# GiboDidact/Computational_ray_tracer

Hardware: AMD Instinct MI355X
Metric: Msamples/s (whole node) at 1920x1080; achieved HBM GB/s vs roofline (higher is better)
Workload: dtype f32; 1 GPU; BASELINE configs[1]: Cornell box 1920x1080 @ 256 spp (16x16 stratified jittered), diffuse + NEE, max depth 5, 1 quad light, 36 triangles; spp_total=256, max_depth=5, parallelism=pixel-tile shards x1 (32x32 tiles) + RCCL film reduce

## Files before the change

### computational_ray_tracer_amd/csrc/rt_device.h

```cpp
#pragma once
#include <hip/hip_runtime.h>
#include <stdint.h>

#include "rt_internal.h"
#include "rt_mathf.h"

namespace rtmi {

#define RT_DEV __device__ __forceinline__

RT_DEV void sincos_det(float x, float& s, float& c) {
    float k = __builtin_rintf(x * 0.636619772367581343f);
    float r = __builtin_fmaf(-k, 1.57079637050628662109375f, x);
    r = __builtin_fmaf(-k, -4.37113900018624283e-8f, r);
    float r2 = r * r;
    float sp = __builtin_fmaf(__builtin_fmaf(-1.9515295891e-4f, r2, 8.3321608736e-3f), r2, -1.6666654611e-1f);
    float sr = __builtin_fmaf(sp * r2, r, r);
    float cp = __builtin_fmaf(__builtin_fmaf(2.443315711809948e-5f, r2, -1.388731625493765e-3f), r2, 4.166664568298827e-2f);
    float cr = __builtin_fmaf(cp * r2, r2, __builtin_fmaf(-0.5f, r2, 1.0f));
    int q = (int)k & 3;
    s = q == 0 ? sr : (q == 1 ? cr : (q == 2 ? -sr : -cr));
    c = q == 0 ? cr : (q == 1 ? -sr : (q == 2 ? -cr : sr));
}
template <class T = rtm::TabConst>
// ... 146 lines not shown
    const uint32_t lo = (uint32_t)delta, hi = (uint32_t)(delta >> 32);
    const uint32_t lo0 = __builtin_amdgcn_readfirstlane(lo), hi0 = __builtin_amdgcn_readfirstlane(hi);
    if (__ballot(lo != lo0 || hi != hi0) == 0) {
        uint64_t d = (uint64_t)lo0 | ((uint64_t)hi0 << 32), M = 1u, P = 0u;
        for (int i = 0; d > 0; ++i, d >>= 1) {
            if (d & 1) {
                const uint64_t cm = kPcgJump.mult[i];
                M *= cm;
                P = P * cm + kPcgJump.plus[i];
            }
        }
        state = M * state + inc * P;
        return;
    }
    uint64_t accMult = 1u, accPlus = 0u;
    for (int i = 0; delta > 0; ++i, delta >>= 1) {
        if (delta & 1) {
            const uint64_t cm = kPcgJump.mult[i];
            accMult *= cm;
            accPlus = accPlus * cm + inc * kPcgJump.plus[i];
        }
    }
    state = accMult * state + accPlus;
}

RT_DEV uint64_t hash_int2(int a, int b) {
    const uint64_t m = 0xc6a4a7935bd1e995ull;
    uint64_t h = 0ull ^ (8ull * m);
    h = murmur_mix_block(h, (uint64_t)(uint32_t)a | ((uint64_t)(uint32_t)b << 32));
    return murmur_final(h);
}
RT_DEV float sobol_sample(const DevSampler& S, uint64_t a, int dimension, int randomize, uint32_t seed) {
    uint32_t v = 0;
    const uint32_t* C = S.sobol_mats + dimension * kSobolMatrixSize;
    for (int i = 0; a != 0; a >>= 1, i++)
        if (a & 1) v ^= C[i];
    if (randomize == 1) {
        v ^= seed;
    } else if (randomize == 2) {
        v = __builtin_bitreverse32(v);
        v ^= v * 0x3d20adeau;
        v += seed;
        v *= (seed >> 16) | 1u;
        v ^= v * 0x05526c56u;
        v ^= v * 0x53a22864u;
        v = __builtin_bitreverse32(v);
// ... 457 lines not shown
```

### computational_ray_tracer_amd/csrc/rt_host.cpp

```cpp
#include <algorithm>
#include <cstddef>
#include <cstdlib>
#include <cmath>
#include <cstdio>
#include <cstring>
#include <limits>
#include <queue>
#include <string>
#include <thread>
#include <utility>
#include <vector>

#include "../../include/rtmi355x.h"
#include "../data/spectra_data.h"
#include "../data/sensor_data.h"
#include "rt_devbuf.h"
#include "rt_guard.h"
#include "rt_internal.h"

using namespace rtmi;

namespace {

constexpr int kRingMax = 1 << 16;
// ... 428 lines not shown
    hipStream_t stream = nullptr;
    hipEvent_t film_done = nullptr;
};

struct Knobs {
    bool stage_events = true;
    int lanes = kDefaultLanes;
    int shadow_queue = 0;
    int shadow_dfs = 1;
    int sort_rays = 1;
    float bvh_node_cost = 2.5f;
    int bvh_max_leaf = kBvhMaxLeaf;
    float bvh_any_cost = 2.f;
    int bvh_any_leaf = 4;
    int force_amb = -1;
    int coop = 1;
    int mat_bins = 1;
    int emit_filter = 1;
    int debug_path = 0;
    int sort_dir_bits = 3, sort_org_bits = 3;
    int sort_org_major = -1;
    int sort_nee = 1, sort_nee_bits = 8;
    int hit_compact = 1;
    size_t batch_samples = 0;
    int denoise_lds = 1;
};

static Knobs read_knobs() {
    Knobs k;
    if (std::getenv("RTMI_NO_STAGE_EVENTS")) k.stage_events = false;
    if (const char* e = std::getenv("RTMI_LANES")) k.lanes = std::max(1, std::min(kLanes, std::atoi(e)));
    if (const char* e = std::getenv("RTMI_SHADOW_QUEUE")) k.shadow_queue = std::atoi(e);
    if (const char* e = std::getenv("RTMI_SHADOW_DFS")) k.shadow_dfs = std::atoi(e);
    if (const char* e = std::getenv("RTMI_SORT")) k.sort_rays = std::atoi(e);
    if (const char* e = std::getenv("RTMI_BVH_CI")) k.bvh_node_cost = (float)std::atof(e);
    if (const char* e = std::getenv("RTMI_BVH_LEAF")) k.bvh_max_leaf = std::max(1, std::min(15, std::atoi(e)));
    if (const char* e = std::getenv("RTMI_BVH_ANY")) {
        float ac;
        int al;
        if (std::sscanf(e, "%f/%d", &ac, &al) == 2) {
            k.bvh_any_cost = ac;
            k.bvh_any_leaf = std::max(1, std::min(15, al));
        }
    }
    if (const char* e = std::getenv("RTMI_FORCE_AMB")) k.force_amb = std::max(-1, std::min(30, std::atoi(e)));
    if (const char* e = std::getenv("RTMI_COOP")) k.coop = std::atoi(e) != 0;
    if (const char* e = std::getenv("RTMI_MAT_BINS")) k.mat_bins = std::atoi(e);
    if (const char* e = std::getenv("RTMI_EMIT_FILTER")) k.emit_filter = std::atoi(e);
    if (const char* e = std::getenv("RTMI_DEBUG_PATH_KERNELS")) k.debug_path = std::atoi(e) != 0;
    if (const char* e = std::getenv("RTMI_SORT_BITS")) {
        int db = 3, ob = 4, om = -1;
        const int got = std::sscanf(e, "%d/%d/%d", &db, &ob, &om);
        if (got >= 2 && db >= 0 && db <= 9 && ob >= 0 && ob <= 9 && 3 + 2 * db + 3 * ob <= 32) {
            k.sort_dir_bits = db;
            k.sort_org_bits = ob;
            if (got == 3) k.sort_org_major = om < 0 ? -1 : (om ? 1 : 0);
        }
    }
    if (const char* e = std::getenv("RTMI_SORT_NEE")) std::sscanf(e, "%d/%d", &k.sort_nee, &k.sort_nee_bits);
    k.sort_nee_bits = std::max(1, std::min(9, k.sort_nee_bits));
    if (const char* e = std::getenv("RTMI_HIT_COMPACT")) k.hit_compact = std::atoi(e) != 0;
    if (const char* e = std::getenv("RTMI_BATCH_SAMPLES")) k.batch_samples = (size_t)std::max(0L, std::atol(e));
    if (const char* e = std::getenv("RTMI_DENOISE_LDS")) k.denoise_lds = std::atoi(e) != 0;
    return k;
}

struct rt_ctx {
    float4 sort_lo{}, sort_scale{};
    int device = 0;
    int octree_build = RT_OCTREE_BUILD_DEVICE;
    hipStream_t stream = nullptr;
    std::string err;
    bool have_scene = false, have_cam = false, have_smp = false, have_film = false, have_integ = false;
    rt_camera_desc cam{};
    rt_sampler_desc smp{};
    rt_film_desc film{};
    rt_integrator_desc integ{};
    int n_tris = 0;
    std::vector<float> h_bounds;
    std::vector<int32_t> h_child, h_leaf_first, h_leaf_count, h_refs;
    rt_octree_info info{};
    bool cull = false;
    bool scene_full = false;
    DevScene dsc{};
// ... 151 lines not shown
    if (path) {
        HIPCHK(c, b.rec.reserve((size_t)kRecF4 * n));
        if (hit_d) HIPCHK(c, b.hitD.reserve(n));
    } else {
        HIPCHK(c, b.lamA.reserve(n)); HIPCHK(c, b.lamB.reserve(n));
    }
    return RT_OK;
}

static int dim_get2d(const DevSampler& S, int dim) {
    if (S.kind == 1) return dim + 2;
    if (S.kind == 2) return (dim + 1 >= kSobolDims ? 2 : dim) + 2;
    return dim;
}
static int dim_after_camera(const DevSampler& S, const DevCamera& cam) {
    int dim = S.kind == 2 ? 2 : 0;
    if (S.kind == 1) dim += 1;
    else if (S.kind == 2) dim = (dim >= kSobolDims ? 2 : dim) + 1;
    if (S.kind == 1) dim += 2;
    if ((cam.type == RT_CAMERA_PERSPECTIVE && cam.lens_radius > 0) || cam.type > RT_CAMERA_PINHOLE)
        dim = dim_get2d(S, dim);
    return dim;
}

hipEvent_t ev_get(rt_ctx* c) {
    if (!c->pool.empty()) {
        hipEvent_t e = c->pool.back();
        c->pool.pop_back();
        return e;
    }
    hipEvent_t e;
    hipEventCreate(&e);
    return e;
}
void ev_mark(rt_ctx* c, hipStream_t st, int stage, hipEvent_t a) {
    if (!a) return;
    hipEvent_t b = ev_get(c);
    hipEventRecord(b, st);
    c->pending.push_back({a, b, stage});
}
hipEvent_t ev_start(rt_ctx* c, hipStream_t st) {
    if (!c->knobs.stage_events) return nullptr;
    hipEvent_t a = ev_get(c);
    hipEventRecord(a, st);
    return a;
}
// ... 330 lines not shown
    }
    const bool dyn = c->dsc.qcap != 1;
    const int lean = c->dsc.full ? 2 : 1;
    const bool shq = c->dsc.qcap != 1 && !c->dsc.full;
    if (shq)
        for (int l = 0; l < lanes; ++l)
            if ((rc = ensure_shadow_workspace(c, c->ws[l].b, ncap))) return rc;
    const bool nee = c->dsc.full && c->dsc.n_lights > 0;
    if (nee)
        for (int l = 0; l < lanes; ++l)
            if ((rc = ensure_nee_workspace(c, c->ws[l].b, nmax * (size_t)nee_stride(c->dsc.n_lights), ncap))) return rc;
    const bool bins = nee && c->dsc.qcap != 1 && kn.mat_bins;
    const int grid = c->grid;
    auto lstream = [&](int l) { return l == 0 ? st : c->ws[l].stream; };
    if (lanes > 1) {
        HIPCHK(c, hipEventRecord(c->ws[0].film_done, st));
        for (int l = 1; l < lanes; ++l) HIPCHK(c, hipStreamWaitEvent(c->ws[l].stream, c->ws[0].film_done, 0));
    }
    const size_t qs = ncap;
    const bool records = c->dsc.qcap != 1;
    const size_t rec_fs = records ? 1 : nmax;
    const unsigned rec_ss = records ? (unsigned)kRecF4 : 1u;
    const int rec_rng8 = !records && lean == 1 ? 1 : 0;
    int last_film = -1;
    for (int g0 = ib; g0 < ie; g0 += B * lanes) {
        int nIdx[kLanes] = {0}, cur[kLanes] = {0}, nSq[kLanes] = {0}, Sq[kLanes] = {0};
        for (int l = 0; l < lanes; ++l) {
            int b0 = g0 + l * B;
            if (b0 >= ie) break;
            Work& w = c->ws[l];
            const Batch& b = w.b;
            hipStream_t s = lstream(l);
            const RecView rv{b.rec.get(), rec_fs, rec_ss, rec_rng8};
            nIdx[l] = std::min(B, ie - b0);
            int nS = nIdx[l] * n_work;
            nSq[l] = nS;
            Sq[l] = shard_stride(nS, nsh);
            SampleIds ids = sample_ids(work, n_work, b0);
            GenOut go{b.rayO(), b.rayD(), nullptr, nullptr, b.pdfA.get(), b.pdfB.get(), rv, lean, 1};
            go.zero = w.qcount.get();
            hipEvent_t e0 = ev_start(c, s);
            HIPCHK(c, launch_generate(s, grid, nS, ids, cam, smp, fd, go));
            ev_mark(c, s, ST_GEN, e0);
        }
        for (int depth = 0; depth <= c->integ.max_depth; ++depth) {
            if (depth == c->integ.max_depth && depth > 0 && !c->dsc.full) break;
            for (int l = 0; l < lanes && nIdx[l] > 0; ++l) {
                Work& w = c->ws[l];
                const Batch& b = w.b;
                hipStream_t s = lstream(l);
                const RecView rv{b.rec.get(), rec_fs, rec_ss, rec_rng8};
                SampleIds ids = sample_ids(work, n_work, g0 + l * B);
                int nxt = cur[l] ^ 1;
                const float4* cO = b.rayO() + 2 * (size_t)cur[l] * qs;
                const float4* cD = cO + 1;
                int* qc_cur = w.qcount.get() + kQRegion * cur[l];
                int* qc_nxt = w.qcount.get() + kQRegion * nxt;
                const bool efilter = kn.emit_filter && c->dsc.full && depth == c->integ.max_depth && depth > 0 &&
                                     c->dsc.n_emit_tris >= 0;
                if (efilter) HIPCHK(c, hipMemsetAsync(qc_nxt, 0, kQRegion * sizeof(int), s));
                hipEvent_t e0;
                QueueView qv = depth == 0 ? QueueView{nullptr, Sq[l], nSq[l], nsh}
                                          : QueueView{qc_cur + kQLen, Sq[l], 0, nsh};
                const DevScene dsl = lane_scene(c, w);
                if (efilter) {
                    const EmitIO eio{qv, cO, b.rayO() + 2 * (size_t)nxt * qs, qc_nxt + kQLen};
                    e0 = ev_start(c, s);
                    HIPCHK(c, launch_emitter_filter(s, grid, dsl, eio));
                    ev_mark(c, s, ST_FILTER, e0);
                    cO = eio.nO;
                    cD = cO + 1;
                    qv = QueueView{qc_nxt + kQLen, Sq[l], 0, nsh};
                }
                TraceIO tio{cO, cD, qv, 0, b.hitB.get(), b.hitPrim.get(), dyn ? qc_cur + kQTraceTicket : nullptr, 1};
                if (depth > 0 && !efilter) tio.zero = qc_nxt;
                const bool hitc = kn.hit_compact && c->dsc.qcap == 1 && !c->dsc.full && depth > 0;
                if (hitc) {
                    tio.hq_d = b.hitD.get();
                    tio.hq_len = qc_cur + kQShadowLen;
                }
                if (c->dsc.qcap != 1) {
                    tio.fb_pos = w.tfb.get();
                    tio.fb_len = qc_cur + kQTraceFallback;
                }
                const NeeSlots ns = nee ? b.nee : NeeSlots{};
                BinIO bio{qv, b.hitPrim.get(), {}, qc_cur + kQBinLen};
                for (int cl = 0; cl < kMatClasses; ++cl) bio.idx[cl] = ns.bin[cl];
                if (depth == 0) { bio.rayO = cO; bio.rec = rv; }
                if (sort_rays && depth > 0 && !efilter) {
                    SortRaysIO so{b.sQKey.get(), b.sS.get(), b.sKeys.get(), b.sKeysAlt.get(), b.sVals.get(),
                                  b.sValsAlt.get(), b.sTemp.get(), kn.sort_dir_bits, kn.sort_org_bits, qc_cur + kQLen,
                                  Sq[l]};
                    e0 = ev_start(c, s);
                    HIPCHK(c, launch_sort_rays(s, so));
                    ev_mark(c, s, ST_SORT, e0);
                    tio.perm = b.sS.get();
                    tio.so = b.sRay.get();
                    cO = tio.so; cD = cO + 1;
                }
                e0 = ev_start(c, s);
                HIPCHK(c, launch_trace_closest(s, grid, c->dsc.qcap, dsl, tio, d_ctr));
                if (tio.fb_pos && !c->dsc.coop_ok)
                    HIPCHK(c, launch_trace_fallback(s, grid, c->dsc.qcap, dsl, tio, d_ctr));
                ev_mark(c, s, ST_TRACE, e0);
                PathIO pio{};
                pio.lean = lean;
                pio.rayO = cO; pio.rayD = cD; pio.q = qv;
                pio.hitB = b.hitB.get(); pio.hitPrim = b.hitPrim.get();
                if (hitc) {
                    pio.q = QueueView{tio.hq_len, Sq[l], 0, nsh};
                    pio.hq_d = tio.hq_d;
                }
                pio.nO =b.rayO() + 2 * (size_t)nxt * qs; pio.nD = pio.nO + 1;
                pio.nCount = qc_nxt + kQLen;
                pio.rec = rv; pio.pdfA = b.pdfA.get(); pio.pdfB = b.pdfB.get();
                pio.depth = depth; pio.max_depth = c->integ.max_depth;
                pio.dim = -1;
                if (lean == 1) {
                    pio.dim = dim_after_camera(smp, cam);
                    for (int d = 0; d < depth; ++d) pio.dim = dim_get2d(smp, dim_get2d(smp, pio.dim));
                }
                pio.ticket = dyn ? qc_cur + kQShadeTicket : nullptr;
                if (sort_rays && depth < c->integ.max_depth) {
                    pio.nkey.key = b.sQKey.get();
                    pio.nkey.lo = c->sort_lo;
                    pio.nkey.scale = c->sort_scale;
                    pio.nkey.dir_bits = kn.sort_dir_bits;
                    pio.nkey.org_bits = kn.sort_org_bits;
                    pio.nkey.org_major = kn.sort_org_major >= 0 ? kn.sort_org_major : (c->dsc.full ? 0 : 1);
                }
                ShadowQueueIO sqio{};
                if (shq) {
                    sqio.shO = b.shO.get(); sqio.shD = b.shD.get(); sqio.shLA = b.shLA.get(); sqio.shLB = b.shLB.get();
                    sqio.shCount = qc_cur + kQShadowLen;
                    sqio.shTicket = qc_cur + kQShadowTicket;
                    sqio.defer = kn.shadow_queue ? 0 : 1;
                }
                NeeIO nio{};
                const bool sort_nee = nee && sort_rays && kn.sort_nee;
                if (nee)
                    nio = NeeIO{b.neeRec.get(), ns.queue, qc_cur + kQShadowLen, qc_cur + kQShadowTicket, ns.fallback,
                                qc_cur + kQNeeFallback, sort_nee ? ns.key : nullptr, c->sort_lo, c->sort_scale,
                                kn.sort_nee_bits};
// ... 2140 lines not shown
```

### computational_ray_tracer_amd/csrc/rt_internal.h

```cpp
#pragma once
#include <hip/hip_runtime.h>
#include <stdint.h>

#include <vector>

namespace rtmi {

static const int kSpecN = 471;
static const int kF1Max = 128;

struct DevSpectra {
    float X[kSpecN], Y[kSpecN], Z[kSpecN], D65[kSpecN];
    float f1_lambda[kF1Max], f1_value[kF1Max];
    int f1_n;
    float bk7_lambda[kF1Max], bk7_value[kF1Max];
    int bk7_n;
    float SR[kSpecN], SG[kSpecN], SB[kSpecN];
    float4 SPK[kSpecN];
};

struct DevCamera {
    float r2c[16], c2w[16];
    float lens_radius, focal_distance;
    int type;
// ... 130 lines not shown
    std::vector<float4> nodes;
    std::vector<float> tiles;
    std::vector<int> tid;
    int depth = 0, max_leaf = 0;
};
void build_bvh8(const float* tri9, const int* ids, int n, float pad, float node_cost, BvhData& out,
                int max_leaf = kBvhMaxLeaf);
void bvh_tiles_logical(const float* t9, const int* tid, int n, float* out12);

}


namespace rtmi {

struct SampleIds {
    const int* work_pixels;
    int n_pixels;
    int index_begin;
    const int* ex_pixel;
    const int* ex_index;
    IntDiv np_div;
};

enum { R_LAM = 0, R_BETA = 2, R_L = 4, R_RNG = 6, R_MISC = 7, kRecF4 = 8 };
struct RecView {
    float4* p;
    size_t fs;
    unsigned ss;
    int rng8;
};

struct GenOut {
    float4* rayO; float4* rayD;
    float4* lamA; float4* lamB; float4* pdfA; float4* pdfB;
    RecView rec;
    int lean;
    int rsh = 0;
    int* zero = nullptr;
};

static const int kShards = 8;
static const int kQStride = 64;
enum { kQLen = 0, kQTraceTicket = 1 * kShards * kQStride, kQShadeTicket = 2 * kShards * kQStride,
       kQShadowLen = 3 * kShards * kQStride, kQShadowTicket = 4 * kShards * kQStride,
       kQNeeFallback = 5 * kShards * kQStride,
       kQBinLen = 6 * kShards * kQStride, kQBinTicket = 8 * kShards * kQStride,
       kQTraceFallback = 10 * kShards * kQStride,
       kQRegion = 11 * kShards * kQStride };
static const int kMatClasses = 2;
inline __host__ __device__ int shard_stride(int n, int ns) {
    int s = (n + ns - 1) / ns;
    return (s + 63) & ~63;
}
struct QueueView {
    const int* len;
    int S;
    int n;
    int ns;
};
static const int kBlockThreads = 256;
static const int kClusterTris = 2;

struct TraceIO {
    const float4* rayO; const float4* rayD;
    QueueView q;
    int set;
    float4* hitB;
    int* hitPrim;
    int* ticket = nullptr;
    int rsh = 0;
    const int* perm = nullptr;
    float4* so = nullptr;
    int* fb_pos = nullptr;
    int* fb_len = nullptr;
    int* zero = nullptr;
    float4* hq_d = nullptr;
    int* hq_len = nullptr;
};

struct BinIO {
    QueueView q;
    const int* hitPrim;
    int* idx[kMatClasses];
    int* len;
    const float4* rayO = nullptr;
    RecView rec{};
};
hipError_t launch_bin_materials(hipStream_t st, int grid, const DevScene& sc, const BinIO& io);

struct EmitIO {
    QueueView q;
    const float4* rayO;
    float4* nO;
    int* nCount;
};
hipError_t launch_emitter_filter(hipStream_t st, int grid, const DevScene& sc, const EmitIO& io);

struct ShadeRefIO {
    const int* work_pixels; int n_pixels; int n_index;
    const float4* rayD; const float4* lamA; const float4* lamB; const float4* pdfA; const float4* pdfB;
// ... 2 lines not shown
    float albedo_c2, illum_c2, illum_scale;
    int rsh;
    float2* mom = nullptr;
};

struct RayKeyIO {
    unsigned* key = nullptr;
    float4 lo, scale;
    int dir_bits = 0, org_bits = 0, org_major = 0;
};
struct PathIO {
    const float4* rayO; const float4* rayD; QueueView q;
    const float4* hitB; const int* hitPrim;
    float4* nO; float4* nD; int* nCount;
    RecView rec;
    float4* pdfA; float4* pdfB;
    int depth, max_depth;
    int lean;
    int dim;
    int* ticket;
    RayKeyIO nkey;
    const int* bin_idx = nullptr;
    const float4* hq_d = nullptr;
};

struct ShadowQueueIO {
    float4 *shO = nullptr, *shD = nullptr, *shLA = nullptr, *shLB = nullptr;
    int *shCount = nullptr, *shTicket = nullptr;
    int defer = 0;
};

inline __host__ __device__ int nee_stride(int n_lights) { return 1 + (n_lights + 1) / 2 + (n_lights + 3) / 4; }
enum { N_PO = 0, N_UV = 1 };
struct NeeIO {
    float4* rec;
    int* slot;
    int* len;
    int* ticket;
    int* fb_slot;
    int* fb_len;
    unsigned* key;
    float4 lo, scale; int key_bits;
};

__device__ __forceinline__ unsigned spread3_9(unsigned v) {
    v &= 0x1ffu;
// ... 168 lines not shown
```

### computational_ray_tracer_amd/csrc/rt_kernels.hip

```cpp
#include <hip/hip_runtime.h>

#include <mutex>
#include <type_traits>
#include <unordered_map>

#include "rt_device.h"

namespace rtmi {

static constexpr int kBlock = kBlockThreads;
static constexpr int kLeafChunk = 32;
static constexpr int kLdsQ = 32;
static constexpr int kTriUnroll = 4;
#ifndef RT_BVH_STACK
#define RT_BVH_STACK 16
#endif
static constexpr int kBvhStack = RT_BVH_STACK;
__shared__ uint2 g_bstk[kBvhStack * kBlock];
static_assert(sizeof(uint2) * kBvhStack >= 2 * kLdsQ, "the BFS FIFO lives in the BVH stack's LDS");
#ifndef RT_ANY_STACK
#define RT_ANY_STACK 24
#endif
static constexpr int kAnyStack = RT_ANY_STACK;
__shared__ unsigned g_astk[kAnyStack * kBlock];
// ... 433 lines not shown
}

__global__ void __launch_bounds__(kBlock) __attribute__((amdgpu_waves_per_eu(4))) k_generate(int nS, SampleIds ids, DevCamera cam, DevSampler smp,
                                                     DevFilm film, GenOut out) {
    stage_warp_tables();
    if (out.zero)
        for (int i = blockIdx.x * blockDim.x + threadIdx.x; i < 2 * kQRegion; i += gridDim.x * blockDim.x) out.zero[i] = 0;
    const bool with_pdf = !out.lean;
    for (int s = blockIdx.x * blockDim.x + threadIdx.x; s < nS; s += gridDim.x * blockDim.x) {
        int pixel, index, x, y;
        sample_of(ids, s, pixel, index);
        pixel_xy(film, pixel, x, y);
        Smp sm;
        float lam[8], pdf[8];
        float4 ro, rd;
        camera_sample(cam, smp, film, x, y, index, sm, lam, ro, rd);
#pragma unroll
        for (int i = 0; i < 8; ++i) pdf[i] = with_pdf ? visible_pdf<WarpTab>(lam[i]) : 0.f;
        out.rayO[s << out.rsh] = make_float4(ro.x, ro.y, ro.z, __int_as_float(s));
        out.rayD[s << out.rsh] = rd;
        if (with_pdf) store8(out.pdfA, out.pdfB, s, pdf);
        if (out.rec.p) {
            rstore8(out.rec, s, R_LAM, lam);
            if (out.rec.rng8)
                rng8_state(out.rec)[s] = make_uint2((uint32_t)sm.rng.state, (uint32_t)(sm.rng.state >> 32));
            else
                *reinterpret_cast<uint4*>(recf(out.rec, s, R_RNG)) =
                    make_uint4((uint32_t)sm.rng.state, (uint32_t)(sm.rng.state >> 32), (uint32_t)pixel, 0u);
            if (out.lean != 1)
                *recf(out.rec, s, R_MISC) = make_float4(__int_as_float(sm.dim), 0.f, 0.f, __int_as_float(pixel));
            if (!out.lean) {
                const float one[8] = {1.f, 1.f, 1.f, 1.f, 1.f, 1.f, 1.f, 1.f};
                const float zero[8] = {0.f, 0.f, 0.f, 0.f, 0.f, 0.f, 0.f, 0.f};
                rstore8(out.rec, s, R_BETA, one);
                rstore8(out.rec, s, R_L, zero);
            }
        } else {
            store8(out.lamA, out.lamB, s, lam);
        }
    }
}

__shared__ float4 g_spk[kSpecN];
__device__ __forceinline__ void stage_spectra(const DevSpectra* sp) {
    for (int i = threadIdx.x; i < kSpecN; i += blockDim.x) g_spk[i] = sp->SPK[i];
    __syncthreads();
}
__device__ __forceinline__ float4 spk_query(const DevSpectra* sp, float lambda) {
    long off = (long)roundf(lambda) - 360;
// ... 887 lines not shown
        for (int si = 0; si < sc.n_shapes; ++si) {
            DevShape sh = ldconst(sc.shapes, si);
            V3 ph;
            float th;
            if (shape_isect<CULL>(sh, v3(o4.x, o4.y, o4.z), v3(d4.x, d4.y, d4.z), tm, ph, th)) {
                prim = sc.n_tris + si; b0 = ph.x; b1 = ph.y; b2 = ph.z; t = th; tm = th;
            }
        }
    }
}
template <bool CULL>
__device__ __forceinline__ int finish_closest(const DevScene& sc, const TraceIO& io, int p, float4 o4, float4 d4,
                                              int prim, float b0, float b1, float b2, float t) {
    closest_shapes<CULL>(sc, o4, d4, prim, b0, b1, b2, t);
    io.hitB[p] = make_float4(b0, b1, b2, t);
    io.hitPrim[p] = prim;
    return prim;
}

#ifndef RT_TRACE_KZ
#define RT_TRACE_KZ 1
#endif

template <int QCAP, bool FBL, bool HQ = false>
__global__ void __launch_bounds__(kBlock) RT_WAVES_ATTR(QCAP) k_trace_closest(DevScene sc, TraceIO io, unsigned long long* ctr) {
    stage_scene<QCAP, false>(sc, io.set);
    if (io.zero && blockIdx.x == 0)
        for (int i = threadIdx.x; i < kQRegion; i += blockDim.x) io.zero[i] = 0;
    ctr_t nn = 0, nt = 0, nh = 0, nr = 0, nfb = 0, novf = 0;
    auto trace_one = [&](int p, float4 o4, float4 d4) __attribute__((always_inline)) {
        float b0 = 0, b1 = 0, b2 = 0, t = 0;
        int prim;
        if constexpr (QCAP != 1 && FBL) {
            bool amb = false;
            prim = traverse_bvh<false, RT_TRACE_KZ != 0>(sc, io.set, v3(o4.x, o4.y, o4.z), v3(d4.x, d4.y, d4.z),
                                                         3.402823466e+38f, b0, b1, b2, t, nn, nt, amb);
            if (amb) {
                ++nfb;
                io.fb_pos[atomicAdd(io.fb_len, 1)] = p;
                return;
            }
        } else {
            prim = traverse_any<QCAP, false>(sc, io.set, v3(o4.x, o4.y, o4.z), v3(d4.x, d4.y, d4.z), 3.402823466e+38f,
                                             b0, b1, b2, t, nn, nt, nfb);
        }
        prim = finish_closest<QCAP != 1>(sc, io, p, o4, d4, prim, b0, b1, b2, t);
        nh += prim >= 0;
// ... 2 lines not shown
    if constexpr (HQ) {
        static_assert(QCAP == 1 && kStaticItems == 2, "a chunk's first record is parked, its second appends both");
        __shared__ int hq_lds[2 * (kBlock / 64) + 1];
        const int n = q_len(io.q, 0);
        int k = blockIdx.x * kChunk + (int)threadIdx.x;
        float4 o4 = make_float4(0, 0, 0, 0), d4 = o4;
        if (k < n) { o4 = io.rayO[k << io.rsh]; d4 = io.rayD[k << io.rsh]; }
        float4 rb0 = o4, rd0 = o4;
        for (int c = blockIdx.x; c * kChunk < n; c += gridDim.x) {
#pragma unroll 1
            for (int r = 0; r < kStaticItems; ++r) {
                const int kn = r + 1 < kStaticItems ? k + kBlock : (c + (int)gridDim.x) * kChunk + (int)threadIdx.x;
                float4 on = o4, dn = d4;
                if (kn < n) { on = io.rayO[kn << io.rsh]; dn = io.rayD[kn << io.rsh]; }
                float b0 = 0, b1 = 0, b2 = 0, t = 0;
                int prim = -1;
                if (k < n) {
                    prim = traverse_any<QCAP, false>(sc, io.set, v3(o4.x, o4.y, o4.z), v3(d4.x, d4.y, d4.z),
                                                     3.402823466e+38f, b0, b1, b2, t, nn, nt, nfb);
                    closest_shapes<false>(sc, o4, d4, prim, b0, b1, b2, t);
                    nh += prim >= 0;
                    nr += 1;
                }
                const float4 rb = make_float4(b0, b1, b2, o4.w), rd = make_float4(d4.x, d4.y, d4.z, __int_as_float(prim));
                if (r == 0) {
                    rb0 = rb;
                    rd0 = rd;
                } else {
                    const bool h0 = __float_as_int(rd0.w) >= 0;
                    int p0, p1;
                    block_append2(io.hq_len, h0, prim >= 0, hq_lds, p0, p1);
                    if (h0) { io.hitB[p0] = rb0; io.hq_d[p0] = rd0; }
                    if (prim >= 0) { io.hitB[p1] = rb; io.hq_d[p1] = rd; }
                }
                k = kn; o4 = on; d4 = dn;
            }
        }
    } else if (!io.ticket && io.q.ns == 1) {
        const int n = q_len(io.q, 0);
        auto item = [&](int i) {
            return (blockIdx.x + (i / kStaticItems) * gridDim.x) * kChunk + (i % kStaticItems) * kBlock +
                   (int)threadIdx.x;
        };
        int k = item(0);
        float4 o4 = make_float4(0, 0, 0, 0), d4 = o4;
        if (k < n) { o4 = io.rayO[k << io.rsh]; d4 = io.rayD[k << io.rsh]; }
        for (int i = 1; k < n; ++i) {
// ... 269 lines not shown

__global__ void k_records(DevScene sc, const DevSpectra* sp, DevFilm film, ShadeRefIO sio, RecordIO io) {
    stage_spectra(sp);
    int s = blockIdx.x * blockDim.x + threadIdx.x;
    if (s >= io.n) return;
    float lam[8], pdf[8], L[8], rgb[3];
    load8(io.lamA, io.lamB, s, lam);
    load8(io.pdfA, io.pdfB, s, pdf);
    li_reference(sc, sp, sio, s, lam, L);
    to_sensor_rgb_spk(sp, L, lam, pdf, film.imaging_ratio, rgb);
    float* r = io.out + (size_t)s * io.stride;
    for (int i = 0; i < 8; ++i) { r[i] = lam[i]; r[8 + i] = pdf[i]; }
    float4 o = io.rayO[s << io.rsh], d = io.rayD[s << io.rsh];
    r[16] = o.x; r[17] = o.y; r[18] = o.z; r[19] = d.x; r[20] = d.y; r[21] = d.z;
    int prim = io.hitPrim[s];
    ((int*)r)[22] = prim;
    float4 hb = prim < 0 ? make_float4(0, 0, 0, 0) : io.hitB[s];
    r[23] = hb.x; r[24] = hb.y; r[25] = hb.z; r[26] = hb.w;
    for (int i = 0; i < 8; ++i) r[27 + i] = L[i];
    for (int c = 0; c < 3; ++c) r[35 + c] = gclamp(rgb[c], 0.0f, 1.0f);
    r[38] = 1.0f;
}

__device__ __forceinline__ void restore_sampler(const SampleIds& ids, const DevFilm& film, const PathIO& io, int slot,
                                                Smp& sm, int smp_kind, int smp_seed, int dim_loaded = -1,
                                                int pixel_loaded = -1) {
    uint2 st;
    if (io.rec.rng8) {
        st = rng8_state(io.rec)[slot];
    } else {
        const uint4 rs = *reinterpret_cast<const uint4*>(recf(io.rec, slot, R_RNG));
        st = make_uint2(rs.x, rs.y);
        pixel_loaded = (int)rs.z;
    }
    int pixel, index, x, y;
    if (pixel_loaded >= 0 && !ids.ex_pixel) {
        pixel = pixel_loaded;
        index = ids.index_begin + (ids.np_div.m ? intdiv(slot, ids.np_div) : slot / ids.n_pixels);
    } else {
        sample_of(ids, slot, pixel, index);
    }
    pixel_xy(film, pixel, x, y);
    sm.rng.state = (uint64_t)st.x | ((uint64_t)st.y << 32);
    sm.rng.inc = smp_kind == 2 ? 0ull : (hash_pixel(x, y, smp_seed) << 1u) | 1u;
    sm.px = x; sm.py = y; sm.index = index;
    sm.dim = io.dim >= 0 ? io.dim : dim_loaded >= 0 ? dim_loaded : __float_as_int(recf(io.rec, slot, R_MISC)->x);
}
__device__ __forceinline__ void save_sampler(const PathIO& io, int slot, const Smp& sm, bool store_dim = true) {
    const uint2 st = make_uint2((uint32_t)sm.rng.state, (uint32_t)(sm.rng.state >> 32));
    if (io.rec.rng8) rng8_state(io.rec)[slot] = st;
    else *reinterpret_cast<uint2*>(recf(io.rec, slot, R_RNG)) = st;
    if (io.dim < 0 && store_dim) *reinterpret_cast<int*>(recf(io.rec, slot, R_MISC)) = sm.dim;
}
__device__ __forceinline__ bool cosine_bounce(float u0, float u1, V3 nrm, V3& wi, float& z) {
    float dx, dy;
    disk_concentric(u0, u1, dx, dy);
    z = 1 - dx * dx - dy * dy;
    z = sqrtf(z > 0.f ? z : 0.f);
    if (z == 0) return false;
    float sign = copysignf(1.0f, nrm.z);
    float a = -1 / (sign + nrm.z);
    float b = nrm.x * nrm.y * a;
    V3 ss = v3(1 + sign * (nrm.x * nrm.x) * a, sign * b, -sign * nrm.x);
    V3 tt = v3(b, sign + (nrm.y * nrm.y) * a, -nrm.y);
    wi = vadd(vadd(vmul(ss, dx), vmul(tt, dy)), vmul(nrm, z));
    return true;
}

template <int QCAP, bool HQ = false>
__global__ void __launch_bounds__(kBlock) __attribute__((amdgpu_waves_per_eu(QCAP == 1 ? RT_SHADE1_WAVES : RT_SHADE_WAVES))) k_path_shade(DevScene sc, const DevSpectra* sp, DevSampler smp,
                                                                         DevFilm film, SampleIds ids, PathIO io,
                                                                         unsigned long long* ctr, ShadowQueueIO shq) {
    const float InvPi = 0.31830988618379067154f;
    bool lds_tris = false;
    stage_spectra(sp);
    stage_scene<QCAP>(sc, 0);
    if constexpr (QCAP == 1) lds_tris = stage_tris1(sc);
    __shared__ int lds[2 * (kBlock / 64) + 1];
    __shared__ float4 pend[QCAP == 1 ? 2 * kBlock : 1];
    bool pend0 = false;
    ctr_t snn = 0, snt = 0, nsh = 0, sfb = 0, novf = 0;
    const bool d0 = io.lean && io.depth == 0;
    constexpr bool WAVE = QCAP != 1;
    std::conditional_t<QCAP == 1, QueueItemsOne, QueueItems<WAVE>> items(io.ticket, io.q);
    int qj, qidx;
    bool live;
    while (items.next(qj, qidx, live)) {
        const int k = qj * io.q.S + qidx;
        bool wantShadow = false, wantNext = false, storedL = false;
        float4 nO = make_float4(0, 0, 0, 0), nD = nO;
        V3 so = v3(0, 0, 0), sd = so;
        float stmax = 0.f;
        float Ld[8];
        int slot = -1;
        if (live) {
            int prim;
            float4 hq = make_float4(0, 0, 0, 0), hd = hq;
            if constexpr (HQ) {
                hq = io.hitB[k];
                hd = io.hq_d[k];
                slot = __float_as_int(hq.w);
                prim = __float_as_int(hd.w);
            } else {
                slot = io.depth == 0 ? k : __float_as_int(io.rayO[2 * k].w);
                prim = io.hitPrim[k];
            }
            if (HQ || prim >= 0) {
                float lam[8], beta[8];
                rload8(io.rec, slot, R_LAM, lam);
                if (d0) {
#pragma unroll
                    for (int i = 0; i < 8; ++i) beta[i] = 1.f;
                } else {
                    rload8(io.rec, slot, R_BETA, beta);
                }
                float4 P0, P1, P2, mt;
                if (QCAP == 1 && lds_tris) {
                    P0 = g_tri1[4 * prim]; P1 = g_tri1[4 * prim + 1]; P2 = g_tri1[4 * prim + 2]; mt = g_tri1[4 * prim + 3];
                } else {
                    P0 = sc.triWorld[3 * prim]; P1 = sc.triWorld[3 * prim + 1]; P2 = sc.triWorld[3 * prim + 2];
                    const DevMaterial dm = sc.materials[sc.triMaterial[prim]];
                    mt = make_float4(dm.c0, dm.c1, dm.c2, dm.emit);
                }
                V3 p0 = v3(P0.x, P0.y, P0.z), p1 = v3(P1.x, P1.y, P1.z), p2 = v3(P2.x, P2.y, P2.z);
                V3 ng = vnorm(vcross(vsub(p0, p2), vsub(p1, p2)));
                const float4 d4 = HQ ? hd : io.rayD[2 * k];
                V3 rayd = vnorm(v3(d4.x, d4.y, d4.z));
                if (mt.w > 0) {
                    if (io.depth == 0 && vdot(ng, rayd) < 0) {
                        float L[8];
                        rload8_or_zero(io.rec, slot, R_L, L, d0);
#pragma unroll
                        for (int i = 0; i < 8; ++i) L[i] += beta[i] * (mt.w * d65_query(sp, lam[i]));
                        rstore8(io.rec, slot, R_L, L);
                        storedL = true;
                    }
                } else if (io.depth < io.max_depth) {
                    V3 nrm = ng;
                    if (vdot(nrm, rayd) > 0) nrm = v3(-nrm.x, -nrm.y, -nrm.z);
                    const float4 hb = HQ ? hq : io.hitB[k];
                    V3 p = vadd(vadd(vmul(p0, hb.x), vmul(p1, hb.y)), vmul(p2, hb.z));
                    float off = 1e-4f * (1.0f + max3f(fabsf(p.x), fabsf(p.y), fabsf(p.z)));
                    V3 po = vadd(p, vmul(nrm, off));
                    constexpr bool kLate = QCAP == 1;
                    float R[8], le = 0.f, wgt = 0.f;
                    if constexpr (!kLate) {
#pragma unroll
                        for (int i = 0; i < 8; ++i) R[i] = sigmoid_eval(mt.x, mt.y, mt.z, lam[i]);
                    }
                    Smp sm;
                    restore_sampler(ids, film, io, slot, sm, smp.kind, smp.seed);
                    float u0, u1;
                    sm.get2d(smp, u0, u1);
                    if (sc.n_lights > 0) {
                        const DevLight& Lq = sc.light0;
                        V3 pl = vadd(vadd(v3(Lq.p[0], Lq.p[1], Lq.p[2]), vmul(v3(Lq.e1[0], Lq.e1[1], Lq.e1[2]), u0)),
                                     vmul(v3(Lq.e2[0], Lq.e2[1], Lq.e2[2]), u1));
                        V3 wv = vsub(pl, po);
                        float dist2 = vdot(wv, wv);
                        float dist = sqrtf(dist2);
                        V3 wi = vmul(wv, 1.0f / dist);
                        float cs = vdot(nrm, wi);
                        float cl = -vdot(v3(Lq.n[0], Lq.n[1], Lq.n[2]), wi);
                        if (cs > 0 && cl > 0) {
                            le = sc.materials[Lq.material].emit;
                            float G = (cs * cl) / dist2;
                            wgt = G * Lq.area;
                            if constexpr (!kLate) {
#pragma unroll
                                for (int i = 0; i < 8; ++i)
                                    Ld[i] = ((beta[i] * (R[i] * InvPi)) * (le * d65_query(sp, lam[i]))) * wgt;
                            }
                            wantShadow = true;
                            so = po;
                            sd = wi;
                            stmax = dist * 0.999f;
                        }
                    }
                    if (io.depth + 1 < io.max_depth) {
                        sm.get2d(smp, u0, u1);
                        V3 wi;
                        float z;
                        if (cosine_bounce(u0, u1, nrm, wi, z)) {
                            if constexpr (!kLate) {
#pragma unroll
                                for (int i = 0; i < 8; ++i) beta[i] *= R[i];
                                rstore8(io.rec, slot, R_BETA, beta);
                            }
                            wantNext = true;
                            nO = make_float4(po.x, po.y, po.z, 0.f);
                            nD = make_float4(wi.x, wi.y, wi.z, 0.f);
                        }
                        save_sampler(io, slot, sm);
                    }
                    if constexpr (kLate) {
#pragma unroll
                        for (int i = 0; i < 8; ++i) {
                            const float Ri = sigmoid_eval(mt.x, mt.y, mt.z, lam[i]);
                            Ld[i] = ((beta[i] * (Ri * InvPi)) * (le * d65_query(sp, lam[i]))) * wgt;
                            beta[i] *= Ri;
                        }
                        if (wantNext) rstore8(io.rec, slot, R_BETA, beta);
                    }
                }
            }
        }
        if constexpr (QCAP == 1) {
            nO.w = __int_as_float(slot);
            if (items.r == 1) {
                if (wantNext) { pend[2 * threadIdx.x] = nO; pend[2 * threadIdx.x + 1] = nD; }
                pend0 = wantNext;
            } else {
                int p0, p1;
                block_append2(io.nCount, pend0, wantNext, lds, p0, p1);
                if (pend0) {
                    const float4 o0 = pend[2 * threadIdx.x], d0v = pend[2 * threadIdx.x + 1];
                    io.nO[2 * p0] = o0; io.nD[2 * p0] = d0v;
                    if (io.nkey.key) io.nkey.key[p0] = ray_sort_key(o0, d0v, io.nkey);
                }
                if (wantNext) {
                    io.nO[2 * p1] = nO; io.nD[2 * p1] = nD;
                    if (io.nkey.key) io.nkey.key[p1] = ray_sort_key(nO, nD, io.nkey);
                }
            }
        }
// ... 814 lines not shown
}

hipError_t launch_trace_closest(hipStream_t st, int grid, int qcap, const DevScene& sc, const TraceIO& io,
                                unsigned long long* ctr) {
    int gb = grid_for(io.q.len ? grid * kBlock : io.q.n, grid);
    if (qcap == 0) gb = std::min(gb, sc.ring_threads / kBlock);
    dim3 b(kBlock);
    const bool fbl = io.fb_pos != nullptr;
    if (fbl && (!io.fb_len || qcap == 1)) return hipErrorInvalidValue;
#define RT_TRACE_CASE(Q)                                                                                          \
    case Q:                                                                                                       \
        if (fbl)                                                                                                  \
            hipLaunchKernelGGL((k_trace_closest<Q, true>), dim3(resident_grid(k_trace_closest<Q, true>, gb, grid)), b, \
                               0, st, sc, io, ctr);                                                               \
        else                                                                                                      \
            hipLaunchKernelGGL((k_trace_closest<Q, false>), dim3(resident_grid(k_trace_closest<Q, false>, gb, grid)), \
                               b, 0, st, sc, io, ctr);                                                            \
        break;
    switch (qcap) {
        RT_TRACE_CASE(0)
        case 1:
            if (io.hq_len) {
                if (io.ticket || io.q.ns != 1 || !io.hq_d) return hipErrorInvalidValue;
                hipLaunchKernelGGL((k_trace_closest<1, false, true>), dim3(resident_grid(k_trace_closest<1, false, true>, gb, grid)), b, 0, st, sc, io, ctr);
            } else {
                hipLaunchKernelGGL((k_trace_closest<1, false>), dim3(resident_grid(k_trace_closest<1, false>, gb, grid)), b, 0, st, sc, io, ctr);
            }
            break;
        RT_TRACE_CASE(16)
        default: return hipErrorInvalidValue;
    }
#undef RT_TRACE_CASE
    return hipGetLastError();
}

hipError_t launch_trace_fallback(hipStream_t st, int grid, int qcap, const DevScene& sc, const TraceIO& io,
                                 unsigned long long* ctr) {
    if (!io.fb_pos || !io.fb_len) return hipErrorInvalidValue;
    int gb = std::min(grid > 0 ? grid : 1, kFallbackBlocks);
    if (qcap == 0) gb = std::min(gb, sc.ring_threads / kBlock);
    dim3 b(kBlock);
    switch (qcap) {
        case 0: hipLaunchKernelGGL(k_trace_fallback<0>, dim3(resident_grid(k_trace_fallback<0>, gb, grid)), b, 0, st, sc, io, ctr); break;
        case 16: hipLaunchKernelGGL(k_trace_fallback<16>, dim3(resident_grid(k_trace_fallback<16>, gb, grid)), b, 0, st, sc, io, ctr); break;
        default: return hipErrorInvalidValue;
    }
    return hipGetLastError();
// ... 30 lines not shown
            hipLaunchKernelGGL((k_path_shadow<Q, true>), dim3(resident_grid(k_path_shadow<Q, true>, gb, grid)), b, \
                               0, st, sc, io, shq, ctr);                                                              \
        else                                                                                                     \
            hipLaunchKernelGGL((k_path_shadow<Q, false>), dim3(resident_grid(k_path_shadow<Q, false>, gb, grid)), \
                               b, 0, st, sc, io, shq, ctr);                                                           \
        break;
    switch (qcap) {
        RT_SHADOW_CASE(0)
        RT_SHADOW_CASE(16)
        default: return hipErrorInvalidValue;
    }
#undef RT_SHADOW_CASE
    return hipGetLastError();
}

hipError_t launch_path_shade(hipStream_t st, int grid, int qcap, const DevScene& sc, const DevSpectra* sp,
                             const DevSampler& smp, const DevFilm& film, const SampleIds& ids, const PathIO& io,
                             unsigned long long* ctr, const ShadowQueueIO& shq, const NeeIO& nee, int matclass) {
    int gb = grid > 0 ? grid : 1;
    if (qcap == 0) gb = std::min(gb, sc.ring_threads / kBlock);
    dim3 b(kBlock);
    if (sc.full && sc.n_lights > 0 && !nee.rec) return hipErrorInvalidValue;
    if (!sc.full && qcap != 1 && !shq.shO) return hipErrorInvalidValue;
#define RT_SHADE_CASE(Q)                                                                                         \
    case Q:                                                                                                      \
        if (sc.full && Q != 1 && matclass == 1)                                                                 \
            hipLaunchKernelGGL((k_path_shade_full<Q, 1>), dim3(resident_grid(k_path_shade_full<Q, 1>, gb, grid)), b, 0, \
                               st, sc, sp, smp, film, ids, io, nee);                                             \
        else if (sc.full && Q != 1 && matclass == 2)                                                            \
            hipLaunchKernelGGL((k_path_shade_full<Q, 2>), dim3(resident_grid(k_path_shade_full<Q, 2>, gb, grid)), b, 0, \
                               st, sc, sp, smp, film, ids, io, nee);                                             \
        else if (sc.full)                                                                                        \
            hipLaunchKernelGGL((k_path_shade_full<Q, 0>), dim3(resident_grid(k_path_shade_full<Q, 0>, gb, grid)), b, 0, \
                               st, sc, sp, smp, film, ids, io, nee);                                             \
        else if (Q == 1 && io.hq_d)                                                                              \
            hipLaunchKernelGGL((k_path_shade<1, true>), dim3(resident_grid(k_path_shade<1, true>, gb, grid)), b, 0, \
                               st, sc, sp, smp, film, ids, io, ctr, shq);                                        \
        else                                                                                                     \
            hipLaunchKernelGGL(k_path_shade<Q>, dim3(resident_grid(k_path_shade<Q>, gb, grid)), b, 0, st, sc, sp,  \
                               smp, film, ids, io, ctr, shq);                                                    \
        break;
    switch (qcap) {
        RT_SHADE_CASE(0)
        RT_SHADE_CASE(1)
        RT_SHADE_CASE(16)
        default: return hipErrorInvalidValue;
    }
#undef RT_SHADE_CASE
    return hipGetLastError();
}

hipError_t launch_path_nee(hipStream_t st, int grid, int qcap, const DevScene& sc, const DevSpectra* sp,
                           const PathIO& io, const NeeIO& nee, unsigned long long* ctr) {
    int gb = grid > 0 ? grid : 1;
    if (qcap == 0) gb = std::min(gb, sc.ring_threads / kBlock);
    dim3 b(kBlock);
    if (qcap != 1 && (!nee.fb_slot || !nee.fb_len)) return hipErrorInvalidValue;
    switch (qcap) {
        case 0: hipLaunchKernelGGL((k_path_nee<0, false>), dim3(resident_grid(k_path_nee<0, false>, gb, grid)), b, 0, st, sc, sp, io, nee, ctr); break;
        case 1: hipLaunchKernelGGL((k_path_nee<1, false>), dim3(resident_grid(k_path_nee<1, false>, gb, grid)), b, 0, st, sc, sp, io, nee, ctr); break;
// ... 73 lines not shown
```

Baseline: 2336 Msamples/s.

## Derive PCG state from sample index instead of storing per-path RNG

Stops writing and reading the per-path 8-byte RNG state in the lean path. Shade recomputes the state with a PCG jump-ahead from a host-computed jump plus per-sample index bits, using a wave-uniform fast path. Optionally (off by default), beta is rebuilt from a packed hit-primitive history kept in the ray direction's w instead of being stored, which only works for small scenes. The aim is less HBM traffic per bounce, paid for with extra integer multiplies per shade. Correctness depends on the jump arithmetic exactly matching the draw counts.

```diff
diff --git a/computational_ray_tracer_amd/csrc/rt_device.h b/computational_ray_tracer_amd/csrc/rt_device.h
--- a/computational_ray_tracer_amd/csrc/rt_device.h
+++ b/computational_ray_tracer_amd/csrc/rt_device.h
@@ -192,6 +192,15 @@
         }
     }
     state = accMult * state + accPlus;
+}
+RT_DEV void pcg_jump_indices(uint64_t& M, uint64_t& P, uint32_t n) {
+    for (int i = 16; n > 0; ++i, n >>= 1) {
+        if (n & 1) {
+            const uint64_t cm = kPcgJump.mult[i];
+            M *= cm;
+            P = P * cm + kPcgJump.plus[i];
+        }
+    }
 }
 
 RT_DEV uint64_t hash_int2(int a, int b) {
diff --git a/computational_ray_tracer_amd/csrc/rt_host.cpp b/computational_ray_tracer_amd/csrc/rt_host.cpp
--- a/computational_ray_tracer_amd/csrc/rt_host.cpp
+++ b/computational_ray_tracer_amd/csrc/rt_host.cpp
@@ -474,6 +474,8 @@
     int sort_org_major = -1;
     int sort_nee = 1, sort_nee_bits = 8;
     int hit_compact = 1;
+    int derive_rng = 1;
+    int derive_beta = 0;
     size_t batch_samples = 0;
     int denoise_lds = 1;
 };
@@ -512,6 +514,8 @@
     if (const char* e = std::getenv("RTMI_SORT_NEE")) std::sscanf(e, "%d/%d", &k.sort_nee, &k.sort_nee_bits);
     k.sort_nee_bits = std::max(1, std::min(9, k.sort_nee_bits));
     if (const char* e = std::getenv("RTMI_HIT_COMPACT")) k.hit_compact = std::atoi(e) != 0;
+    if (const char* e = std::getenv("RTMI_DERIVE_RNG")) k.derive_rng = std::atoi(e) != 0;
+    if (const char* e = std::getenv("RTMI_DERIVE_BETA")) k.derive_beta = std::atoi(e) != 0;
     if (const char* e = std::getenv("RTMI_BATCH_SAMPLES")) k.batch_samples = (size_t)std::max(0L, std::atol(e));
     if (const char* e = std::getenv("RTMI_DENOISE_LDS")) k.denoise_lds = std::atoi(e) != 0;
     return k;
@@ -709,6 +713,26 @@
         dim = dim_get2d(S, dim);
     return dim;
 }
+static int draws_get2d(const DevSampler& S) { return S.kind == 0 || (S.kind == 1 && S.jitter) ? 2 : 0; }
+static int draws_after_camera(const DevSampler& S, const DevCamera& cam) {
+    int n = draws_get2d(S) / 2;
+    n += draws_get2d(S);
+    if ((cam.type == RT_CAMERA_PERSPECTIVE && cam.lens_radius > 0) || cam.type > RT_CAMERA_PINHOLE)
+        n += draws_get2d(S);
+    return n;
+}
+static PcgJump pcg_jump(uint64_t delta) {
+    uint64_t cm = 0x5851f42d4c957f2dull, cp = 1, am = 1, ap = 0;
+    for (; delta > 0; delta >>= 1) {
+        if (delta & 1) {
+            am *= cm;
+            ap = ap * cm + cp;
+        }
+        cp = (cm + 1) * cp;
+        cm *= cm;
+    }
+    return PcgJump{am, ap};
+}
 
 hipEvent_t ev_get(rt_ctx* c) {
     if (!c->pool.empty()) {
@@ -1085,6 +1109,9 @@
     const size_t rec_fs = records ? 1 : nmax;
     const unsigned rec_ss = records ? (unsigned)kRecF4 : 1u;
     const int rec_rng8 = !records && lean == 1 ? 1 : 0;
+    const bool derive_rng = kn.derive_rng && lean == 1 && smp.kind != 2 && !(smp.kind == 1 && ie > smp.spp);
+    const bool derive_beta = kn.derive_beta && lean == 1 && c->dsc.qcap == 1 && c->dsc.n_tris <= 64 &&
+                             c->dsc.n_shapes == 0 && c->integ.max_depth <= 5;
     int last_film = -1;
     for (int g0 = ib; g0 < ie; g0 += B * lanes) {
         int nIdx[kLanes] = {0}, cur[kLanes] = {0}, nSq[kLanes] = {0}, Sq[kLanes] = {0};
@@ -1102,6 +1129,7 @@
             SampleIds ids = sample_ids(work, n_work, b0);
             GenOut go{b.rayO(), b.rayD(), nullptr, nullptr, b.pdfA.get(), b.pdfB.get(), rv, lean, 1};
             go.zero = w.qcount.get();
+            go.no_rng = derive_rng ? 1 : 0;
             hipEvent_t e0 = ev_start(c, s);
             HIPCHK(c, launch_generate(s, grid, nS, ids, cam, smp, fd, go));
             ev_mark(c, s, ST_GEN, e0);
@@ -1141,6 +1169,7 @@
                 if (hitc) {
                     tio.hq_d = b.hitD.get();
                     tio.hq_len = qc_cur + kQShadowLen;
+                    tio.hq_hist = derive_beta ? 1 : 0;
                 }
                 if (c->dsc.qcap != 1) {
                     tio.fb_pos = w.tfb.get();
@@ -1182,6 +1211,12 @@
                 if (lean == 1) {
                     pio.dim = dim_after_camera(smp, cam);
                     for (int d = 0; d < depth; ++d) pio.dim = dim_get2d(smp, dim_get2d(smp, pio.dim));
+                }
+                pio.derive_beta = derive_beta ? 1 : 0;
+                if (derive_rng) {
+                    pio.derive_rng = 1;
+                    pio.jump = pcg_jump((uint64_t)ids.index_begin * 65536ull +
+                                        (uint64_t)(draws_after_camera(smp, cam) + 2 * depth * draws_get2d(smp)));
                 }
                 pio.ticket = dyn ? qc_cur + kQShadeTicket : nullptr;
                 if (sort_rays && depth < c->integ.max_depth) {
diff --git a/computational_ray_tracer_amd/csrc/rt_internal.h b/computational_ray_tracer_amd/csrc/rt_internal.h
--- a/computational_ray_tracer_amd/csrc/rt_internal.h
+++ b/computational_ray_tracer_amd/csrc/rt_internal.h
@@ -176,6 +176,9 @@
     IntDiv np_div;
 };
 
+struct PcgJump {
+    unsigned long long mult = 1, plus = 0;
+};
 enum { R_LAM = 0, R_BETA = 2, R_L = 4, R_RNG = 6, R_MISC = 7, kRecF4 = 8 };
 struct RecView {
     float4* p;
@@ -191,6 +194,7 @@
     int lean;
     int rsh = 0;
     int* zero = nullptr;
+    int no_rng = 0;
 };
 
 static const int kShards = 8;
@@ -230,6 +234,7 @@
     int* zero = nullptr;
     float4* hq_d = nullptr;
     int* hq_len = nullptr;
+    int hq_hist = 0;
 };
 
 struct BinIO {
@@ -278,6 +283,9 @@
     RayKeyIO nkey;
     const int* bin_idx = nullptr;
     const float4* hq_d = nullptr;
+    PcgJump jump{};
+    int derive_rng = 0;
+    int derive_beta = 0;
 };
 
 struct ShadowQueueIO {
diff --git a/computational_ray_tracer_amd/csrc/rt_kernels.hip b/computational_ray_tracer_amd/csrc/rt_kernels.hip
--- a/computational_ray_tracer_amd/csrc/rt_kernels.hip
+++ b/computational_ray_tracer_amd/csrc/rt_kernels.hip
@@ -479,9 +479,10 @@
         if (with_pdf) store8(out.pdfA, out.pdfB, s, pdf);
         if (out.rec.p) {
             rstore8(out.rec, s, R_LAM, lam);
-            if (out.rec.rng8)
-                rng8_state(out.rec)[s] = make_uint2((uint32_t)sm.rng.state, (uint32_t)(sm.rng.state >> 32));
-            else
+            if (out.rec.rng8) {
+                if (!out.no_rng)
+                    rng8_state(out.rec)[s] = make_uint2((uint32_t)sm.rng.state, (uint32_t)(sm.rng.state >> 32));
+            } else
                 *reinterpret_cast<uint4*>(recf(out.rec, s, R_RNG)) =
                     make_uint4((uint32_t)sm.rng.state, (uint32_t)(sm.rng.state >> 32), (uint32_t)pixel, 0u);
             if (out.lean != 1)
@@ -1415,7 +1416,7 @@
 #define RT_TRACE_KZ 1
 #endif
 
-template <int QCAP, bool FBL, bool HQ = false>
+template <int QCAP, bool FBL, bool HQ = false, bool HH = false>
 __global__ void __launch_bounds__(kBlock) RT_WAVES_ATTR(QCAP) k_trace_closest(DevScene sc, TraceIO io, unsigned long long* ctr) {
     stage_scene<QCAP, false>(sc, io.set);
     if (io.zero && blockIdx.x == 0)
@@ -1464,7 +1465,8 @@
                     nh += prim >= 0;
                     nr += 1;
                 }
-                const float4 rb = make_float4(b0, b1, b2, o4.w), rd = make_float4(d4.x, d4.y, d4.z, __int_as_float(prim));
+                const int pw = HH && prim >= 0 ? prim | (__float_as_int(d4.w) << 6) : prim;
+                const float4 rb = make_float4(b0, b1, b2, o4.w), rd = make_float4(d4.x, d4.y, d4.z, __int_as_float(pw));
                 if (r == 0) {
                     rb0 = rb;
                     rd0 = rd;
@@ -1780,12 +1782,13 @@
     r[38] = 1.0f;
 }
 
+template <bool DR = false>
 __device__ __forceinline__ void restore_sampler(const SampleIds& ids, const DevFilm& film, const PathIO& io, int slot,
                                                 Smp& sm, int smp_kind, int smp_seed, int dim_loaded = -1,
                                                 int pixel_loaded = -1) {
-    uint2 st;
+    uint2 st = make_uint2(0u, 0u);
     if (io.rec.rng8) {
-        st = rng8_state(io.rec)[slot];
+        if constexpr (!DR) st = rng8_state(io.rec)[slot];
     } else {
         const uint4 rs = *reinterpret_cast<const uint4*>(recf(io.rec, slot, R_RNG));
         st = make_uint2(rs.x, rs.y);
@@ -1800,7 +1803,17 @@
     }
     pixel_xy(film, pixel, x, y);
     sm.rng.state = (uint64_t)st.x | ((uint64_t)st.y << 32);
-    sm.rng.inc = smp_kind == 2 ? 0ull : (hash_pixel(x, y, smp_seed) << 1u) | 1u;
+    if constexpr (DR) {
+        uint64_t M = io.jump.mult, P = io.jump.plus;
+        const uint32_t j = (uint32_t)(index - ids.index_begin), j0 = __builtin_amdgcn_readfirstlane(j);
+        if (__ballot(j != j0) == 0) pcg_jump_indices(M, P, j0);
+        else pcg_jump_indices(M, P, j);
+        const uint64_t seq = hash_pixel(x, y, smp_seed);
+        sm.rng.inc = (seq << 1u) | 1u;
+        sm.rng.state = (M * 0x5851f42d4c957f2dull) * (sm.rng.inc + mix_bits(seq)) + sm.rng.inc * (M + P);
+    } else {
+        sm.rng.inc = smp_kind == 2 ? 0ull : (hash_pixel(x, y, smp_seed) << 1u) | 1u;
+    }
     sm.px = x; sm.py = y; sm.index = index;
     sm.dim = io.dim >= 0 ? io.dim : dim_loaded >= 0 ? dim_loaded : __float_as_int(recf(io.rec, slot, R_MISC)->x);
 }
@@ -1825,7 +1838,7 @@
     return true;
 }
 
-template <int QCAP, bool HQ = false>
+template <int QCAP, bool HQ = false, bool DR = false, bool DB = false>
 __global__ void __launch_bounds__(kBlock) __attribute__((amdgpu_waves_per_eu(QCAP == 1 ? RT_SHADE1_WAVES : RT_SHADE_WAVES))) k_path_shade(DevScene sc, const DevSpectra* sp, DevSampler smp,
                                                                          DevFilm film, SampleIds ids, PathIO io,
                                                                          unsigned long long* ctr, ShadowQueueIO shq) {
@@ -1853,12 +1866,14 @@
         int slot = -1;
         if (live) {
             int prim;
+            int hist = 0;
             float4 hq = make_float4(0, 0, 0, 0), hd = hq;
             if constexpr (HQ) {
                 hq = io.hitB[k];
                 hd = io.hq_d[k];
                 slot = __float_as_int(hq.w);
                 prim = __float_as_int(hd.w);
+                if constexpr (DB) { hist = prim >> 6; prim &= 63; }
             } else {
                 slot = io.depth == 0 ? k : __float_as_int(io.rayO[2 * k].w);
                 prim = io.hitPrim[k];
@@ -1866,7 +1881,7 @@
             if (HQ || prim >= 0) {
                 float lam[8], beta[8];
                 rload8(io.rec, slot, R_LAM, lam);
-                if (d0) {
+                if (DB || d0) {
 #pragma unroll
                     for (int i = 0; i < 8; ++i) beta[i] = 1.f;
                 } else {
@@ -1883,6 +1898,7 @@
                 V3 p0 = v3(P0.x, P0.y, P0.z), p1 = v3(P1.x, P1.y, P1.z), p2 = v3(P2.x, P2.y, P2.z);
                 V3 ng = vnorm(vcross(vsub(p0, p2), vsub(p1, p2)));
                 const float4 d4 = HQ ? hd : io.rayD[2 * k];
+                if constexpr (DB && !HQ) hist = io.depth == 0 ? 0 : __float_as_int(d4.w);
                 V3 rayd = vnorm(v3(d4.x, d4.y, d4.z));
                 if (mt.w > 0) {
                     if (io.depth == 0 && vdot(ng, rayd) < 0) {
@@ -1907,7 +1923,7 @@
                         for (int i = 0; i < 8; ++i) R[i] = sigmoid_eval(mt.x, mt.y, mt.z, lam[i]);
                     }
                     Smp sm;
-                    restore_sampler(ids, film, io, slot, sm, smp.kind, smp.seed);
+                    restore_sampler<DR>(ids, film, io, slot, sm, smp.kind, smp.seed);
                     float u0, u1;
                     sm.get2d(smp, u0, u1);
                     if (sc.n_lights > 0) {
@@ -1947,18 +1963,26 @@
                             }
                             wantNext = true;
                             nO = make_float4(po.x, po.y, po.z, 0.f);
-                            nD = make_float4(wi.x, wi.y, wi.z, 0.f);
+                            nD = make_float4(wi.x, wi.y, wi.z, DB ? __int_as_float(hist | prim << 6 * io.depth) : 0.f);
                         }
-                        save_sampler(io, slot, sm);
+                        if constexpr (!DR) save_sampler(io, slot, sm);
                     }
                     if constexpr (kLate) {
+                        if constexpr (DB) {
+#pragma unroll 1
+                            for (int j = 0; j < io.depth; ++j) {
+                                const float4 mj = g_tri1[4 * ((hist >> 6 * j) & 63) + 3];
+#pragma unroll
+                                for (int i = 0; i < 8; ++i) beta[i] *= sigmoid_eval(mj.x, mj.y, mj.z, lam[i]);
+                            }
+                        }
 #pragma unroll
                         for (int i = 0; i < 8; ++i) {
                             const float Ri = sigmoid_eval(mt.x, mt.y, mt.z, lam[i]);
                             Ld[i] = ((beta[i] * (Ri * InvPi)) * (le * d65_query(sp, lam[i]))) * wgt;
                             beta[i] *= Ri;
                         }
-                        if (wantNext) rstore8(io.rec, slot, R_BETA, beta);
+                        if (!DB && wantNext) rstore8(io.rec, slot, R_BETA, beta);
                     }
                 }
             }
@@ -2819,7 +2843,10 @@
         case 1:
             if (io.hq_len) {
                 if (io.ticket || io.q.ns != 1 || !io.hq_d) return hipErrorInvalidValue;
-                hipLaunchKernelGGL((k_trace_closest<1, false, true>), dim3(resident_grid(k_trace_closest<1, false, true>, gb, grid)), b, 0, st, sc, io, ctr);
+                if (io.hq_hist)
+                    hipLaunchKernelGGL((k_trace_closest<1, false, true, true>), dim3(resident_grid(k_trace_closest<1, false, true, true>, gb, grid)), b, 0, st, sc, io, ctr);
+                else
+                    hipLaunchKernelGGL((k_trace_closest<1, false, true>), dim3(resident_grid(k_trace_closest<1, false, true>, gb, grid)), b, 0, st, sc, io, ctr);
             } else {
                 hipLaunchKernelGGL((k_trace_closest<1, false>), dim3(resident_grid(k_trace_closest<1, false>, gb, grid)), b, 0, st, sc, io, ctr);
             }
@@ -2896,6 +2923,9 @@
     dim3 b(kBlock);
     if (sc.full && sc.n_lights > 0 && !nee.rec) return hipErrorInvalidValue;
     if (!sc.full && qcap != 1 && !shq.shO) return hipErrorInvalidValue;
+    if (io.derive_beta && (sc.full || qcap != 1 || sc.n_tris > 64 || sc.n_shapes != 0 || io.max_depth > 5))
+        return hipErrorInvalidValue;
+    if (io.derive_rng && (sc.full || io.dim < 0)) return hipErrorInvalidValue;
 #define RT_SHADE_CASE(Q)                                                                                         \
     case Q:                                                                                                      \
         if (sc.full && Q != 1 && matclass == 1)                                                                 \
@@ -2907,9 +2937,27 @@
         else if (sc.full)                                                                                        \
             hipLaunchKernelGGL((k_path_shade_full<Q, 0>), dim3(resident_grid(k_path_shade_full<Q, 0>, gb, grid)), b, 0, \
                                st, sc, sp, smp, film, ids, io, nee);                                             \
+        else if (Q == 1 && io.derive_beta && io.hq_d && io.derive_rng)                                           \
+            hipLaunchKernelGGL((k_path_shade<1, true, true, true>), dim3(resident_grid(k_path_shade<1, true, true, true>, gb, grid)), \
+                               b, 0, st, sc, sp, smp, film, ids, io, ctr, shq);                                  \
+        else if (Q == 1 && io.derive_beta && io.hq_d)                                                            \
+            hipLaunchKernelGGL((k_path_shade<1, true, false, true>), dim3(resident_grid(k_path_shade<1, true, false, true>, gb, grid)), \
+                               b, 0, st, sc, sp, smp, film, ids, io, ctr, shq);                                  \
+        else if (Q == 1 && io.derive_beta && io.derive_rng)                                                      \
+            hipLaunchKernelGGL((k_path_shade<1, false, true, true>), dim3(resident_grid(k_path_shade<1, false, true, true>, gb, grid)), \
+                               b, 0, st, sc, sp, smp, film, ids, io, ctr, shq);                                  \
+        else if (Q == 1 && io.derive_beta)                                                                       \
+            hipLaunchKernelGGL((k_path_shade<1, false, false, true>), dim3(resident_grid(k_path_shade<1, false, false, true>, gb, grid)), \
+                               b, 0, st, sc, sp, smp, film, ids, io, ctr, shq);                                  \
+        else if (Q == 1 && io.hq_d && io.derive_rng)                                                             \
+            hipLaunchKernelGGL((k_path_shade<1, true, true>), dim3(resident_grid(k_path_shade<1, true, true>, gb, grid)), \
+                               b, 0, st, sc, sp, smp, film, ids, io, ctr, shq);                                  \
         else if (Q == 1 && io.hq_d)                                                                              \
             hipLaunchKernelGGL((k_path_shade<1, true>), dim3(resident_grid(k_path_shade<1, true>, gb, grid)), b, 0, \
                                st, sc, sp, smp, film, ids, io, ctr, shq);                                        \
+        else if (io.derive_rng)                                                                                  \
+            hipLaunchKernelGGL((k_path_shade<Q, false, true>), dim3(resident_grid(k_path_shade<Q, false, true>, gb, grid)), \
+                               b, 0, st, sc, sp, smp, film, ids, io, ctr, shq);                                  \
         else                                                                                                     \
             hipLaunchKernelGGL(k_path_shade<Q>, dim3(resident_grid(k_path_shade<Q>, gb, grid)), b, 0, st, sc, sp,  \
                                smp, film, ids, io, ctr, shq);                                                    \
```

Result: faster. 2370 Msamples/s, median of 6 (+1.4%).
